# xyfJASON/diffusion-models-pytorch

Measured on AMD Instinct MI355X. Metric: images/sec at DDIM-50, CIFAR-10 UNet 32×32, bs=256; 1/2/4/8 GPU, higher is better.
Workload: dtype f32 via fp16x2 split MFMA

## Files before the change

diffusion-models-pytorch_amd/csrc/api.hip:

```cpp
#include <algorithm>
#include <cstdlib>
#include <cstring>
#include <string>
#include "dm_common.h"
#include "dm_kernels.h"

namespace dm {
namespace {
thread_local std::string g_last_error;
}
void set_error(const std::string& msg) { g_last_error = msg; }
const char* last_error() { return g_last_error.c_str(); }

namespace {
thread_local Toggles t_toggles;
thread_local const Toggles* t_scope = nullptr;
bool env_is(const char* name, char c) {
  const char* e = std::getenv(name);
  return e && e[0] == c;
}
bool g_launch_log_on = false;
bool g_launch_log_convs = false;
std::string g_launch_log;
}
// ... 16 lines not shown
  t.k32_small = !env_is("DM_CONV_K32S", '0');
  t.k32_s2 = !env_is("DM_CONV_K32S2", '0');
  t.k32_t2d = !env_is("DM_CONV_K32T2", '0');
  t.k32_8x = !env_is("DM_K32_8X", '0');
  t.gn_fusion = !env_is("DM_GN_FUSION", '0');
  if (const char* e = std::getenv("DM_ATTN")) {
    const std::string v(e);
    t.attn = v == "3" ? 3 : v == "0" || v == "presplit" ? 0 : v == "noproj" ? kAttnNoProj : v == "fused" ? kAttnFused
           : v == "unfused" ? kAttnUnfused : 4;
  }
  t.attn_gn_launch = env_is("DM_ATTN_GNFIN", '1');
  t.attn_small = !env_is("DM_ATTN_SMALL", '0');
  t.dit_presplit = !env_is("DM_DIT_PRESPLIT", '0');
  t.lin_sk = !env_is("DM_LIN_SK", '0');
  t.lin_rows = !env_is("DM_LIN_ROWS", '0');
  t_toggles = t;
}
void note_launch(const char* name) {
  if (!g_launch_log_on) return;
  g_launch_log += name;
  g_launch_log += '\n';
}
}

extern "C" int dm_debug_launch_log(int enable) {
  dm::g_launch_log_on = enable != 0;
  dm::g_launch_log_convs = enable == 2;
  if (enable) dm::g_launch_log.clear();
  return DM_OK;
}
// ... 309 lines not shown
```

diffusion-models-pytorch_amd/csrc/dm_kernels.h:

```cpp
#pragma once
#include <cstdlib>
#include <string>
#include "dm_common.h"

namespace dm {

constexpr int kGnPixPerChunk = 64;

constexpr int kAttnNoProj = 1, kAttnFused = 2, kAttnUnfused = 5;
struct Toggles {
  int conv_math = 2;
  bool range_check = true;
  bool graph = true;
  bool wino = true;
  bool k32s_w4 = false;
  bool k32_small = true;
  bool k32_s2 = true;
  bool k32_t2d = true;
  bool k32_8x = true;
  bool gn_fusion = true;
  int attn = 4;
  bool attn_gn_launch = false;
  bool attn_small = true;
  bool dit_presplit = true;
  bool lin_sk = true;
  bool lin_rows = true;
};
const Toggles& toggles();
void refresh_toggles();
const Toggles* toggle_scope_swap(const Toggles* t);
struct ToggleScope {
  const Toggles* prev;
  explicit ToggleScope(const Toggles& t) : prev(toggle_scope_swap(&t)) {}
  ~ToggleScope() { toggle_scope_swap(prev); }
  ToggleScope(const ToggleScope&) = delete;
  ToggleScope& operator=(const ToggleScope&) = delete;
};
void note_launch(const char* name);

constexpr int kPickBatch = 256;

// ... 340 lines not shown
```

diffusion-models-pytorch_amd/csrc/unet_exec.hip:

```cpp
#include <memory>
#include <vector>
#include <functional>
#include <cmath>
#include <map>
#include <set>

#include "dm_common.h"
#include "dm_kernels.h"
#include "plan.h"
#include "exec_pack.h"
#include "exec_core.h"

namespace dm {

namespace {

struct GnP { size_t g, b; int C; };
struct ConvP {
  size_t w, bias;
  int Cout, Cin, taps, K;
  size_t w_sub = 0;
};

struct ResBlockP {
// ... 50 lines not shown
  std::vector<AttnP> attn;
  std::vector<ConvP> convs;
  std::vector<Node> nodes;
  std::vector<int> skip_C, skip_level;
  int n_levels = 0;
  float norm_eps = 1e-5f;

  struct Plan : PlanBase {
    int B = 0, H = 0, W = 0;
    int math = 0;
    bool half = false;
    float* x = nullptr;
    int64_t* t = nullptr;
    int64_t* y = nullptr;
    float* out = nullptr;
  };
  PlanCache<Plan> plans;
  float* last_packed = nullptr;
  using FoldW = AttnFoldW;
  std::map<size_t, FoldW> folds;
  std::vector<void*> fold_mem;
  const FoldW* fold_for(const AttnP& p);

  UNetModel() { wino_small = true; }
  ~UNetModel() {
    for (void* q : fold_mem) (void)hipFree(q);
    if (last_packed) (void)hipFree(last_packed);
  }
  int build_plan(Plan& pl, int B, int H, int W);
  int get_plan(int B, int H, int W, int math, Plan** out) {
    conv_math = math;
    const bool half = half_active();
    return plans.get([&](const Plan& p) { return p.B == B && p.H == H && p.W == W && p.math == math && p.half == half; },
                     [&](Plan& p) { return build_plan(p, B, H, W); }, out);
  }
};

const UNetModel::FoldW* UNetModel::fold_for(const AttnP& p) {
  auto it = folds.find(p.wqkv);
  if (it != folds.end()) return it->second.at ? &it->second : nullptr;
  const int C = p.C;
  FoldW f;
  void* mem = nullptr;
  const size_t nb = attn_fold_bytes(C);
  if (hipMalloc(&mem, nb) != hipSuccess) {
    (void)hipGetLastError();
    folds[p.wqkv] = FoldW{};
    return nullptr;
  }
  fold_mem.push_back(mem);
  const double s = (double)p.sa * (p.sb != 0.f ? (double)p.sb : 1.0);
  if (attn_fold_all(P(p.wqkv), P(p.bqkv), P(p.wproj), P(p.bproj), C, s, mem, &f, nullptr) != DM_OK ||
      hipDeviceSynchronize() != hipSuccess) {
    folds[p.wqkv] = FoldW{};
    return nullptr;
  }
  split_bytes += nb - 64;
  return &(folds[p.wqkv] = f);
}

static int first_channels(const dm_unet_arch& a) { return a.variant == 2 ? a.dim * a.dim_mults[0] : a.dim; }

static int attn_heads(const dm_unet_arch& a, int C, int where) {
  if (a.variant == 3) return 1;
  if (a.variant == 2) {
    if (a.attn_head_dims > 0) return C / a.attn_head_dims;
    return where == 2 ? a.n_heads_up : a.n_heads;
  }
  if (where == 1) return 1;
  return a.variant == 1 ? C / a.attn_head_dims : a.n_heads;
}

static int count_params(const dm_unet_arch& a) {
// ... 385 lines not shown
  auto alloc = [&](size_t bytes) -> float* { return pl.alloc(bytes); };
  auto Hl = [&](int lvl) { return H >> lvl; };
  auto Wl = [&](int lvl) { return W >> lvl; };
  const int D = arch.dim, TD = 4 * arch.dim, G = 32, C0 = skip_C[0];
  const float gn_eps = norm_eps;

  pl.x = alloc((size_t)B * arch.in_channels * H * W * 4);
  pl.t = (int64_t*)alloc((size_t)B * 8);
  pl.y = (int64_t*)alloc((size_t)B * 8);
  pl.out = alloc((size_t)B * arch.out_channels * H * W * 4);
  float* e0 = alloc((size_t)B * D * 4);
  float* e1 = alloc((size_t)B * TD * 4);
  float* se = alloc((size_t)B * TD * 4);
  float* e2 = has_class ? alloc((size_t)B * TD * 4) : nullptr;
  float* projs = alloc((size_t)B * proj_total * 4);

  size_t max_a1 = 0, max_h = 0, max_attn = 0, max_qkv = 0, max_S = 0, max_xr = 0;
  int max_chunks = 1;
  for (auto& n : nodes) {
    const size_t hw = (size_t)Hl(n.level_in) * Wl(n.level_in);
    max_chunks = std::max(max_chunks, gn_num_chunks((int)hw));
    if (n.kind == N_RES) {
      const size_t hw_o = (size_t)Hl(n.level_out) * Wl(n.level_out);
      max_chunks = std::max(max_chunks, gn_num_chunks((int)hw_o));
      max_a1 = std::max(max_a1, (size_t)B * std::max(hw, hw_o) * n.cin);
      max_h = std::max(max_h, (size_t)B * hw_o * n.cout);
      if (res[n.idx].updown) max_xr = std::max(max_xr, (size_t)B * hw_o * n.cin);
    } else if (n.kind == N_ATTN) {
      max_attn = std::max(max_attn, (size_t)B * hw * n.cin);
      max_qkv = std::max(max_qkv, (size_t)B * hw * 3 * n.cin);
// ... 107 lines not shown
    conv_cost(c, fl, by);
    add(conv_label(c), fl, by, [=](hipStream_t st) { return conv2d_igemm(c, st); });
  };
  auto add_gemm = [&](const GemmArgs& g) {
    double fl, by;
    gemm_cost(g, fl, by);
    add(gemm_label(g), fl, by, [=](hipStream_t st) { return gemm_batched(g, st); });
  };
  auto gn_bytes = [](const View& v, bool apply) {
    const double n = (double)v.B * v.H * v.W * v.C;
    return apply ? 8.0 * n : 4.0 * n;
  };
  Plan* P_ = &pl;
  UNetModel* self = this;

  add("timestep_embed", 0, 4.0 * B * D, [=](hipStream_t st) {
    return timestep_embed(P_->t, B, D, self->arch.variant == 2 ? 1 : 0,
                          self->freqs_set ? self->P(self->freqs) : nullptr, e0, st);
  });
  auto add_rows = [&](const GemmArgs& g) {
    const long tiles64 = (long)ceil_div(kPickBatch, 64) * ceil_div(g.N, 64);
    if (!toggles().lin_rows || !linear_rows_ok(g) || tiles64 >= 256) return add_gemm(g);
    double fl, by;
    gemm_cost(g, fl, by);
    add("linear_rows_kernel", fl, by, [=](hipStream_t st) { return linear_rows(g, st); });
  };
  {
    GemmArgs g{};
    g.M = B; g.N = TD; g.K = D; g.Z1 = 1; g.Z2 = 1; g.pick_M = kPickBatch;
    g.A = e0; g.lda = D; g.Bm = P(te_w1); g.ldb = D; g.C = e1; g.ldc = TD; g.alpha = 1.f;
// ... 5 lines not shown
    if (has_class) {
      g2.act = 0;
      g2.C = e2;
      add_rows(g2);
      const float* table = P(class_embed);
      add("class_embed_silu", 0, 8.0 * B * TD, [=](hipStream_t st) {
        return embed_add_silu(e2, P_->y, table, B, TD, se, st);
      });
    } else {
      add_rows(g2);
    }
    GemmArgs g3 = g;
    g3.N = proj_total; g3.K = TD; g3.A = se; g3.lda = TD; g3.Bm = P(proj_w); g3.ldb = TD; g3.C = projs;
    g3.ldc = proj_total; g3.bias = P(proj_b); g3.act = 0;
    add_rows(g3);
  }

  auto out_view_for = [&](int i, int C, int lvl) -> View {
    if (i >= 0 && nodes[i].skip_producer) return skip_view[nodes[i].skip_id];
    const int nx = i + 1;
    if (nx < (int)nodes.size() && nodes[nx].kind == N_RES && nodes[nx].pops_skip >= 0) return concat_x[nx];
    float* buf = alloc((size_t)B * Hl(lvl) * Wl(lvl) * C * 4);
    return View{buf, B, Hl(lvl), Wl(lvl), C, C};
  };

  struct GnReady {
    double2* p;
    int C, G;
  };
  std::map<const float*, GnReady> gn_ready;
// ... 115 lines not shown
      View vh{hbuf, B, Ho, Wo, r.cout, r.cout};
      View va2{a2, B, Ho, Wo, r.cout, r.cout};
      View xres = xin;
      if (r.updown) {
        xres = View{xr, B, Ho, Wo, r.cin, r.cin};
        const bool down = r.updown == 2;
        add("resample2x", 0, 4.0 * B * ((double)Hi * Wi + (double)Ho * Wo) * r.cin,
            [=](hipStream_t st) { return resample2x(xin, xres, down, nullptr, nullptr, st); });
      }
      ConvArgs c1{};
      c1.x1_pitch = r.cin; c1.Cin1 = r.cin; c1.Hin = Ho; c1.Win = Wo;
      c1.taps = 9; c1.stride = 1; c1.upsample = 0;
      c1.w = P(r.conv1.w); c1.K = r.conv1.K;
      c1.y = hbuf; c1.y_pitch = r.cout; c1.Cout = r.cout; c1.B = B; c1.pick_B = kPickBatch; c1.Hout = Ho; c1.Wout = Wo;
      c1.bias = P(r.conv1.bias);
      if (!r.adagn) { c1.rowvec = projs + r.proj_col; c1.rowvec_pitch = proj_total; }
      if (r.updown == 1) { c1.upsample = 1; c1.Hin = Hi; c1.Win = Wi; }
      auto try_subpix = [&](ConvArgs& c, size_t w_sub) {
        if (!c.upsample || !w_sub) return;
        ConvArgs s = c;
        s.upsample = 2; s.w = P(w_sub); s.K = 4 * c.Cin1;
        split_for(s);
        if (conv_pick(s) >= 3) c = s;
      };
      ConvArgs c2{};
      c2.x1 = a2; c2.x1_pitch = r.cout; c2.Cin1 = r.cout; c2.Hin = Ho; c2.Win = Wo;
      c2.taps = 9; c2.stride = 1;
      c2.w = P(r.conv2.w); c2.K = r.conv2.K;
      c2.y = y.p; c2.y_pitch = y.pitch; c2.Cout = r.cout; c2.B = B; c2.pick_B = kPickBatch; c2.Hout = Ho; c2.Wout = Wo;
      c2.bias = P(r.conv2.bias);
      if (r.cin != r.cout) {
        c2.x2 = xres.p; c2.x2_pitch = xres.pitch; c2.Cin2 = r.cin;
      } else {
        c2.res = xres.p; c2.res_pitch = xres.pitch;
      }
      split_for(c1);
      split_for(c2);
      try_subpix(c1, r.conv1.w_sub);
      const bool fuse1 = r.updown != 2 && conv_pick(c1) >= 3, fuse2 = conv_pick(c2) >= 3;
      const float* ms = r.adagn ? projs + r.proj_col : nullptr;
      const float* mb = r.adagn ? projs + r.proj_col + r.cout : nullptr;
      const int mp = r.adagn ? proj_total : 0;
      const double2* st1 = n.pops_skip >= 0 ? gn_stats_concat(xin, skip_view[n.pops_skip]) : gn_stats(xin);
      if (r.updown && !fuse1) {
        add("gn_finalize", 0, 8.0 * B * r.cin, [=](hipStream_t st) {
          return gn_finalize(xin, G, st1, gn_eps, self->P(r.gn1.g), self->P(r.gn1.b), gsc, gsh, st);
        });
        const bool down = r.updown == 2;
        add("resample2x", 0, 4.0 * B * ((double)Hi * Wi + (double)Ho * Wo) * r.cin,
            [=](hipStream_t st) { return resample2x(xin, va1, down, gsc, gsh, st); });
        c1.x1 = a1; c1.upsample = 0; c1.Hin = Ho; c1.Win = Wo;
        c1.w = P(r.conv1.w); c1.K = r.conv1.K;
      } else if (fuse1) {
        c1.x1 = xin.p; c1.x1_pitch = xin.pitch;
        gn_prologue(c1, xin, st1, r.gn1.g, r.gn1.b, nullptr, nullptr, 0);
      } else {
        add("gn_apply", 0, gn_bytes(xin, true), [=](hipStream_t st) {
// ... 305 lines not shown
    for (int i = 0; i < n; ++i) order[i] = i;
  }
  return DM_OK;
}

extern "C" int dm_unet_create(const dm_unet_arch* arch, const float* const* params, const int64_t* numels,
                              int n_params, void* stream, dm_unet** out) {
  if (!out || !params || !numels) { dm::set_error("null argument"); return DM_ERR_ARG; }
  dm::UNetModel* m = nullptr;
  int rc = dm::unet_create(arch, params, numels, n_params, (hipStream_t)stream, &m);
  if (rc) return rc;
  *out = new dm_unet{m};
  return DM_OK;
}

extern "C" int dm_unet_forward(dm_unet* h, const float* x, const int64_t* t, const int64_t* y, int B, int H, int W,
                               float* out, void* stream) {
  dm::UNetModel* m = dm::model_of(h);
  DM_ABI_MODEL(m);
  if (!x || !t || !out) { dm::set_error("null tensor"); return DM_ERR_ARG; }
  if (B <= 0 || H <= 0 || W <= 0) { dm::set_error("empty batch or image"); return DM_ERR_ARG; }
  if (static_cast<const void*>(out) == static_cast<const void*>(x)) {
    dm::set_error("out must not alias x");
    return DM_ERR_ARG;
  }
  hipStream_t st = (hipStream_t)stream;
  const size_t nx = (size_t)B * m->arch.in_channels * H * W, no = (size_t)B * m->arch.out_channels * H * W;
  using Plan = dm::UNetModel::Plan;
  return dm::run_forward(
      *m, st, [&](int math, Plan** pl) { return m->get_plan(B, H, W, math, pl); },
      [&](Plan& pl) {
        DM_CHECK_HIP(hipMemcpyAsync(pl.x, x, nx * sizeof(float), hipMemcpyDeviceToDevice, st));
        DM_CHECK_HIP(hipMemcpyAsync(pl.t, t, (size_t)B * sizeof(int64_t), hipMemcpyDeviceToDevice, st));
        if (m->has_class) {
          if (y)
            DM_CHECK_HIP(hipMemcpyAsync(pl.y, y, (size_t)B * sizeof(int64_t), hipMemcpyDeviceToDevice, st));
          else
            DM_CHECK_HIP(hipMemsetAsync(pl.y, 0xff, (size_t)B * sizeof(int64_t), st));
        }
        return DM_OK;
      },
      [&](Plan& pl) {
        DM_CHECK_HIP(hipMemcpyAsync(out, pl.out, no * sizeof(float), hipMemcpyDeviceToDevice, st));
        return DM_OK;
      });
}

extern "C" int dm_unet_set_range_deferred(dm_unet* h, int deferred) {
  return dm::abi_set_range_deferred(dm::model_of(h), deferred);
}
extern "C" int dm_unet_range_poll(dm_unet* h, void* stream, int* flagged) {
  return dm::abi_range_poll(dm::model_of(h), (hipStream_t)stream, flagged);
}
extern "C" int dm_unet_range_fallback(dm_unet* h, int on) { return dm::abi_range_fallback(dm::model_of(h), on); }
extern "C" int dm_unet_range_stats(const dm_unet* h, int64_t* fallbacks, int* active) {
  return dm::abi_range_stats(dm::model_of(h), fallbacks, active);
}
extern "C" int dm_unet_memory(const dm_unet* h, int64_t* weight_bytes, int64_t* workspace_bytes) {
  return dm::abi_memory(dm::model_of(h), weight_bytes, workspace_bytes);
}

extern "C" int dm_unet_share_workspace(dm_unet* a, dm_unet* b) {
  if (!a || !a->m || !b || !b->m) { dm::set_error("null model"); return DM_ERR_STATE; }
  if (a->m->plans.pool != b->m->plans.pool) b->m->plans.share(a->m->plans.pool);
  return DM_OK;
}

extern "C" int dm_unet_plan_stats(const dm_unet* h, int64_t* builds, int* cached) {
  return dm::abi_plan_stats(dm::model_of(h), builds, cached);
}
extern "C" int dm_unet_set_conv_math(dm_unet* h, int kind) { return dm::abi_set_math(dm::model_of(h), kind, true); }
extern "C" int dm_unet_get_conv_math(const dm_unet* h, int* kind) { return dm::abi_get_math(dm::model_of(h), kind); }

extern "C" int dm_unet_set_conv_half(dm_unet* h, int on) {
  auto* m = dm::model_of(h);
  DM_ABI_MODEL(m);
  if (on != 0 && on != 1) { dm::set_error("conv_half must be 0 or 1"); return DM_ERR_ARG; }
  if ((on != 0) != m->conv_half) {
    m->conv_half = on != 0;
    m->plans.clear();
  }
  return DM_OK;
}
extern "C" int dm_unet_get_conv_half(const dm_unet* h, int* on) {
  auto* m = dm::model_of(h);
  DM_ABI_MODEL(m && on);
  *on = m->conv_half ? 1 : 0;
  return DM_OK;
}
extern "C" int dm_unet_set_time_freqs(dm_unet* h, const float* freqs, int n, void* stream) {
  return dm::abi_set_time_freqs(dm::model_of(h), freqs, n, (hipStream_t)stream);
}
extern "C" int dm_unet_profile(dm_unet* h, int enable) { return dm::abi_profile(dm::model_of(h), enable); }
extern "C" int dm_unet_profile_count(dm_unet* h, int* n_ops) { return dm::abi_profile_count(dm::model_of(h), n_ops); }
extern "C" int dm_unet_profile_get(dm_unet* h, int i, char* label, int label_len, double* flops, double* bytes,
                                   double* ms_total, int64_t* launches) {
  return dm::abi_profile_get(dm::model_of(h), i, label, label_len, flops, bytes, ms_total, launches);
}
extern "C" void dm_unet_destroy(dm_unet* h) { dm::abi_destroy(h); }
```

diffusion-models-pytorch_amd/diffusions/ddim.py:

```python
from typing import Any, Dict

import torch
import tqdm
from torch import Tensor

from diffusions.ddpm import DDPM, _CFGMixin


class DDIM(DDPM):
    kind = 0

    def __init__(
            self,
            total_steps: int = 1000,
            beta_schedule: str = 'linear',
            beta_start: float = 0.0001,
            beta_end: float = 0.02,
            betas: Tensor = None,
            objective: str = 'pred_eps',

            clip_denoised: bool = True,
            respace_type: str = None,
            respace_steps: int = 100,
            respaced_seq: Tensor = None,
# ... 34 lines not shown
        if self.eta != 0.:
            raise ValueError(f'DDIM inversion is only valid when eta=0, get {self.eta}')
        out = self._step(model_output, xt, t, 0, model_output_uncond=model_output_uncond,
                         guidance_scale=guidance_scale, want_noise=False, coefs=self._inversion_coefs(t, t_next))
        return {'sample': out['sample'], 'pred_x0': out['pred_x0'], 'pred_eps': out['pred_eps']}

    def sample_inversion_loop(
            self, model, img: Tensor,
            tqdm_kwargs: Dict = None, model_kwargs: Dict = None,
    ):
        tqdm_kwargs = dict() if tqdm_kwargs is None else tqdm_kwargs
        model_kwargs = dict() if model_kwargs is None else model_kwargs
        seq = self.respaced_seq.tolist()
        pbar = tqdm.tqdm(total=len(seq) - 1, **tqdm_kwargs)
        for t, t_next in zip(seq[:-1], seq[1:]):
            t_batch = torch.full((img.shape[0], ), t, device=img.device, dtype=torch.long)
            model_output = model(img, t_batch, **model_kwargs)
            out = self.denoise_inversion(model_output, img, t, t_next)
            img = out['sample']
            pbar.update(1)
            yield out
        pbar.close()

    def sample_inversion(
            self, model, img: Tensor,
            tqdm_kwargs: Dict = None, model_kwargs: Dict = None,
    ):
        sample = None
        for out in self.sample_inversion_loop(model, img, tqdm_kwargs, model_kwargs):
            sample = out['sample']
        return sample

# ... 40 lines not shown
```

diffusion-models-pytorch_amd/diffusions/ddpm.py:

```python
import math
from contextlib import contextmanager
from typing import Any, Callable, Dict, Optional

import torch
import tqdm
from torch import Tensor

import dmhip
from diffusions.schedule import get_beta_schedule, get_respaced_seq

_OBJECTIVES = {'pred_eps': 0, 'pred_x0': 1, 'pred_v': 2}
_VAR_TYPES = ('fixed_small', 'fixed_large', 'learned_range')


class DDPM:
    kind = 1

    def __init__(
            self,
            total_steps: int = 1000,
            beta_schedule: str = 'linear',
            beta_start: float = 0.0001,
            beta_end: float = 0.02,
            betas: Tensor = None,
            objective: str = 'pred_eps',

            var_type: str = 'fixed_large',
# ... 214 lines not shown

    def denoise(self, model_output: Tensor, xt: Tensor, t: int, t_prev: int):
        return self._step(model_output, xt, t, t_prev)

    def sample_loop(
            self, model, init_noise: Tensor,
            tqdm_kwargs: Dict = None, model_kwargs: Dict = None,
    ):
        tqdm_kwargs = dict() if tqdm_kwargs is None else tqdm_kwargs
        model_kwargs = dict() if model_kwargs is None else model_kwargs
        img = init_noise
        seq = self.respaced_seq.tolist()
        seq_prev = [-1] + seq[:-1]
        pbar = tqdm.tqdm(total=len(seq), **tqdm_kwargs)
        for t, t_prev in zip(reversed(seq), reversed(seq_prev)):
            t_batch = torch.full((img.shape[0], ), t, device=img.device, dtype=torch.long)
            model_output = model(img, t_batch, **model_kwargs)
            out = self.denoise(model_output, img, t, t_prev)
            img = out['sample']
            pbar.update(1)
            yield out
        pbar.close()

    def sample(
            self, model, init_noise: Tensor,
            tqdm_kwargs: Dict = None, model_kwargs: Dict = None,
    ):
        def run():
            sample = None
            for out in self.sample_loop(model, init_noise, tqdm_kwargs, model_kwargs):
                sample = out['sample']
            return sample
# ... 87 lines not shown
```

diffusion-models-pytorch_amd/diffusions/heun.py:

```python
from typing import Dict

import torch
import tqdm
from torch import Tensor

from diffusions.euler import EulerSampler


class HeunSampler(EulerSampler):
    def __init__(self, *args, **kwargs):
        super().__init__(*args, **kwargs)
        self._1st_order_derivative = None
        self._1st_order_xt = None

    def denoise_1st_order(self, model_output: Tensor, xt: Tensor, t: int, t_prev: int):
        derivative = torch.empty_like(xt)
        out = self._first_order(model_output, xt, t, t_prev, derivative=derivative)
        self._1st_order_derivative = derivative
        self._1st_order_xt = xt
        return {'sample': out['sample'], 'pred_x0': out['pred_x0']}

    def denoise_2nd_order(self, model_output: Tensor, xt_prev: Tensor, t: int, t_prev: int):
        if self._1st_order_derivative is None:
            raise RuntimeError('denoise_2nd_order needs a preceding denoise_1st_order')
# ... 5 lines not shown
        self._1st_order_derivative = None
        self._1st_order_xt = None
        return {'sample': out['sample'], 'pred_x0': out['pred_x0']}

    def sample_loop(
            self, model, init_noise: Tensor,
            tqdm_kwargs: Dict = None, model_kwargs: Dict = None,
    ):
        tqdm_kwargs = dict() if tqdm_kwargs is None else tqdm_kwargs
        model_kwargs = dict() if model_kwargs is None else model_kwargs
        img = init_noise
        seq = self.respaced_seq.tolist()
        seq_prev = [-1] + seq[:-1]
        pbar = tqdm.tqdm(total=len(seq), **tqdm_kwargs)
        for t, t_prev in zip(reversed(seq), reversed(seq_prev)):
            t_batch = torch.full((img.shape[0], ), t, device=img.device, dtype=torch.long)
            model_output = model(img, t_batch, **model_kwargs)
            out = self.denoise_1st_order(model_output, img, t, t_prev)
            img = out['sample']
            if t_prev >= 0:
                t_prev_batch = torch.full((img.shape[0], ), t_prev, device=img.device, dtype=torch.long)
                model_output = model(img, t_prev_batch, **model_kwargs)
                out = self.denoise_2nd_order(model_output, img, t, t_prev)
                img = out['sample']
            pbar.update(1)
            yield out
        pbar.close()
```

diffusion-models-pytorch_amd/dmhip/__init__.py:

```python
from dmhip._lib import (
    DMError,
    lib,
    lib_path,
    load,
    exported_symbols,
    require_device_tensor,
    stream_handle,
    StepDesc,
    ConvDesc,
    GemmDesc,
    UNetArch,
    DiTArch,
    VaeArch,
    VaeEncArch,
    sampler_step,
    groupnorm_nhwc,
    groupnorm_affine,
    conv2d_nhwc,
    conv2d_nhwc_s2pad0,
    conv2d_gn_stats,
    pack_conv_weight,
    pack_conv_weight_subpixel,
    pack_conv_weight_split,
    pack_conv_weight_wino,
# ... 8 lines not shown
    SPLIT_BF16X3,
    MATH_FP16,
    MATH_NAMES,
    TOKEN_MATH,
    gemm,
    softmax_rows,
    timestep_embedding,
    unet_profile_enable,
    unet_profile_read,
    null_label_scope,
    null_labels_allowed,
    deferred_range_check,
    plan_stats,
    range_stats,
    share_workspace,
    lincomb,
    GuideDesc,
    guided_step,
    LowpassPlan,
)
```

diffusion-models-pytorch_amd/dmhip/_lib.py:

```python
import ctypes
import os
import re
from typing import Optional

import torch

_HERE = os.path.dirname(os.path.abspath(__file__))
lib_path = os.environ.get('DM_HIP_LIB') or os.path.join(_HERE, 'libdm_hip.so')
_HEADER = os.path.join(os.path.dirname(os.path.dirname(_HERE)), 'include', 'dm_hip.h')

ABI_VERSION = 2
DM_OK = 0
DM_ERR_ARG = -1
DM_ERR_HIP = -2
DM_ERR_STATE = -3
DM_ERR_UNSUPPORTED = -4
DM_MAX_STAGES = 8


class DMError(RuntimeError):
    """A failure reported by the native library (HIP error, bad state)."""


c_float_p = ctypes.POINTER(ctypes.c_float)
# ... 191 lines not shown

    def end_fallback(self):
        for handle, abi in self.flagged_handles:
            check(getattr(load(), abi + '_range_fallback')(handle, 0), abi + '_range_fallback')
        self.flagged_handles = []


def _declare(L: ctypes.CDLL):
    L.dm_abi_version.restype = ctypes.c_int
    L.dm_last_error.restype = ctypes.c_char_p
    L.dm_build_info.restype = ctypes.c_char_p
    L.dm_unet_param_count.argtypes = [ctypes.POINTER(UNetArch), ctypes.POINTER(ctypes.c_int)]
    L.dm_unet_create.argtypes = [ctypes.POINTER(UNetArch), ctypes.POINTER(vp), ctypes.POINTER(ctypes.c_int64),
                                 ctypes.c_int, vp, ctypes.POINTER(vp)]
    L.dm_unet_forward.argtypes = [vp, vp, vp, vp, ctypes.c_int, ctypes.c_int, ctypes.c_int, vp, vp]
    L.dm_unet_profile.argtypes = [vp, ctypes.c_int]
    L.dm_unet_profile_count.argtypes = [vp, ctypes.POINTER(ctypes.c_int)]
    L.dm_unet_profile_get.argtypes = [vp, ctypes.c_int, ctypes.c_char_p, ctypes.c_int,
                                      ctypes.POINTER(ctypes.c_double), ctypes.POINTER(ctypes.c_double),
                                      ctypes.POINTER(ctypes.c_double), ctypes.POINTER(ctypes.c_int64)]
    L.dm_unet_memory.argtypes = [vp, ctypes.POINTER(ctypes.c_int64), ctypes.POINTER(ctypes.c_int64)]
    L.dm_unet_destroy.argtypes = [vp]
    L.dm_unet_destroy.restype = None
    L.dm_sampler_step.argtypes = [ctypes.POINTER(StepDesc), vp]
    L.dm_groupnorm_scratch_bytes.argtypes = [ctypes.c_int, ctypes.c_int, ctypes.c_int]
    L.dm_groupnorm_scratch_bytes.restype = ctypes.c_int64
    L.dm_groupnorm_nhwc.argtypes = [vp, ctypes.c_int, vp, ctypes.c_int, ctypes.c_int, ctypes.c_int, ctypes.c_int,
                                    ctypes.c_int, ctypes.c_float, vp, vp, vp, vp, ctypes.c_int, ctypes.c_int, vp, vp]
    L.dm_groupnorm_affine.argtypes = [vp, ctypes.c_int, ctypes.c_int, ctypes.c_int, ctypes.c_int, ctypes.c_int,
                                      ctypes.c_float, vp, vp, vp, vp, vp, vp]
# ... 391 lines not shown


def range_stats(handle, abi: str = 'dm_unet'):
    n, active = ctypes.c_int64(), ctypes.c_int()
    check(getattr(load(), abi + '_range_stats')(handle, ctypes.byref(n), ctypes.byref(active)), abi + '_range_stats')
    return n.value, {v: k for k, v in MATH_NAMES.items()}[active.value]


def plan_stats(handle, abi: str = 'dm_unet'):
    builds, cached = ctypes.c_int64(), ctypes.c_int()
    check(getattr(load(), abi + '_plan_stats')(handle, ctypes.byref(builds), ctypes.byref(cached)),
          abi + '_plan_stats')
    return builds.value, cached.value


def share_workspace(a, b):
    check(load().dm_unet_share_workspace(a, b), 'dm_unet_share_workspace')


def lincomb(mode: int, a: torch.Tensor, b: torch.Tensor, c1, c2, out: torch.Tensor = None) -> torch.Tensor:
    for name, t in (('a', a), ('b', b)):
        require_device_tensor(t, name)
    if a.shape != b.shape:
        raise ValueError(f'lincomb: shapes {tuple(a.shape)} and {tuple(b.shape)} differ')
    if out is None:
        out = torch.empty_like(a)
    else:
        require_device_tensor(out, 'out')
        if out.shape != a.shape:
            raise ValueError(f'lincomb: out has shape {tuple(out.shape)}, the operands {tuple(a.shape)}')
# ... 34 lines not shown
```

diffusion-models-pytorch_amd/models/pesser/model.py:

```python
from typing import Sequence

import torch.nn as nn
from torch import Tensor

from ..unet import ConvHalf, NativeDenoiser


def _gn(C: int) -> nn.GroupNorm:
    return nn.GroupNorm(32, C, eps=1e-6)


def _conv(cin: int, cout: int, k: int, stride: int = 1, padding: int = None) -> nn.Conv2d:
    return nn.Conv2d(cin, cout, k, stride=stride, padding=k // 2 if padding is None else padding)


def _holder(**children) -> nn.Module:
    m = nn.Module()
    for name, child in children.items():
        m.add_module(name, child)
    return m


class ResnetBlock(nn.Module):

# ... 13 lines not shown
    def __init__(self, C: int):
        super().__init__()
        self.norm = _gn(C)
        for name in ('q', 'k', 'v', 'proj_out'):
            self.add_module(name, _conv(C, C, 1))


class Resample(nn.Module):

    def __init__(self, C: int, down: bool):
        super().__init__()
        self.conv = _conv(C, C, 3, stride=2, padding=0) if down else _conv(C, C, 3)


class Model(ConvHalf, NativeDenoiser):
    def __init__(self, *, ch: int, out_ch: int, ch_mult: Sequence[int] = (1, 2, 4, 8), num_res_blocks: int,
                 attn_resolutions: Sequence[int], dropout: float = 0.0, resamp_with_conv: bool = True,
                 in_channels: int, resolution: int):
        super().__init__()
        if not resamp_with_conv:
            raise NotImplementedError('resamp_with_conv=False (average-pool / nearest resampling without convs) is '
                                      'used by no shipped config and is not built')
        self.ch = ch
        self.resolution = resolution
        self.in_channels = in_channels
        listed = {int(r) for r in attn_resolutions}
        widths = [ch * int(m) for m in ch_mult]
        n_levels = len(widths)
        use_attn = [(resolution >> lvl) in listed for lvl in range(n_levels)]
        self.arch = dict(in_channels=in_channels, out_channels=out_ch, dim=ch, dim_mults=[int(m) for m in ch_mult],
# ... 23 lines not shown
                           block_2=ResnetBlock(cur, cur, embed))

        ups = {}
        for lvl in reversed(range(n_levels)):
            cins = []
            for _ in range(num_res_blocks + 1):
                cins.append(cur + skips.pop())
                cur = widths[lvl]
            ups[lvl] = stage(lvl, cins, dict(upsample=Resample(cur, down=False)) if lvl else {})
        assert not skips
        self.up = nn.ModuleList(ups[lvl] for lvl in range(n_levels))

        self.norm_out = _gn(cur)
        self.conv_out = _conv(cur, out_ch, 3)

    def forward(self, x: Tensor, t: Tensor):
        if tuple(x.shape[2:]) != (self.resolution, self.resolution):
            raise AssertionError(f'expected {self.resolution} x {self.resolution} images, got {tuple(x.shape[2:])}')
        return self._run(x, t)
```

diffusion-models-pytorch_amd/models/unet.py:

```python
import ctypes
import math
from typing import List, Sequence

import torch
import torch.nn as nn
from torch import Tensor

import dmhip
from dmhip._lib import UNetArch, check, load, stream_handle


def _gn(C: int) -> nn.GroupNorm:
    return nn.GroupNorm(32, C)


def _conv(cin: int, cout: int, k: int, stride: int = 1) -> nn.Conv2d:
    return nn.Conv2d(cin, cout, k, stride=stride, padding=k // 2)


class ResBlock(nn.Module):

    def __init__(self, in_channels: int, out_channels: int, embed_dim: int, dropout: float = 0.1):
        super().__init__()
        self.blk1 = nn.Sequential(_gn(in_channels), nn.SiLU(), _conv(in_channels, out_channels, 3))
# ... 17 lines not shown
        self.scale = (dim // n_heads) ** -0.5


class _TimeEmbedding(nn.Sequential):

    def __init__(self, dim: int):
        super().__init__(nn.Identity(), nn.Linear(dim, 4 * dim), nn.SiLU(), nn.Linear(4 * dim, 4 * dim))


class NativeDenoiser(nn.Module):

    _native = None
    _native_key = None
    _param_list = None
    _abi = 'dm_unet'

    def _arch_struct(self) -> UNetArch:
        a = UNetArch()
        a.in_channels = self.arch['in_channels']
        a.out_channels = self.arch['out_channels']
        a.dim = self.arch['dim']
        a.n_stages = len(self.arch['dim_mults'])
        for i, (m, at) in enumerate(zip(self.arch['dim_mults'], self.arch['use_attn'])):
            a.dim_mults[i] = m
            a.use_attn[i] = int(at)
        a.num_res_blocks = self.arch['num_res_blocks']
        a.n_heads = self.arch.get('n_heads', 1)
        a.variant = self.arch.get('variant', 0)
        a.num_classes = self.arch.get('num_classes', 0) or 0
        a.attn_head_dims = self.arch.get('attn_head_dims', 0)
# ... 55 lines not shown
        if peer is not None and self._abi == 'dm_unet' and getattr(peer, '_abi', None) == 'dm_unet' \
                and getattr(peer, '_native', None) is not None:
            dmhip.share_workspace(peer._native, handle)

    def _time_freqs(self) -> Tensor:
        half = self.arch['dim'] // 2
        if self.arch.get('variant', 0) == 2:
            return torch.exp(-math.log(10000) * torch.arange(start=0, end=half, dtype=torch.float32) / half)
        return torch.exp(torch.arange(half) * -(math.log(10000) / (half - 1)))

    def _launch(self, handle, X: Tensor, T: Tensor, y_ptr, out: Tensor):
        B, _, H, W = X.shape
        check(load().dm_unet_forward(handle, X.data_ptr(), T.data_ptr(), y_ptr, B, H, W, out.data_ptr(),
                                     stream_handle(X.device)), 'dm_unet_forward')

    def _apply(self, fn, *args, **kwargs):
        self._release_native()
        return super()._apply(fn, *args, **kwargs)

    def __del__(self):
        try:
            self._release_native()
        except Exception:
            pass

    def _run(self, X: Tensor, T: Tensor, y: Tensor = None) -> Tensor:
        dmhip.require_device_tensor(X, 'X')
        dmhip.require_device_tensor(T, 'T', dtype=torch.long)
        if X.ndim != 4 or X.shape[1] != self.arch['in_channels']:
            raise ValueError(f'expected input [B, {self.arch["in_channels"]}, H, W], got {tuple(X.shape)}')
        B, _, H, W = X.shape
        if T.shape != (B, ):
            raise ValueError(f'expected T of shape ({B},), got {tuple(T.shape)}')
        y_ptr = None
        if y is not None:
            dmhip.require_device_tensor(y, 'y', dtype=torch.long)
            if y.shape != (B, ):
                raise ValueError(f'expected y of shape ({B},), got {tuple(y.shape)}')
            self._check_labels(y)
            y_ptr = y.data_ptr()
        handle = self.native_handle(X.device)
        scope = dmhip.deferred_range_check.active
        if scope is not None:
            scope.register(handle, self._abi, X.device)
        out = torch.empty((B, self.arch['out_channels'], H, W), device=X.device, dtype=torch.float32)
        self._launch(handle, X, T, y_ptr, out)
        return out

    def _check_labels(self, y: Tensor):
        null_ok = dmhip.null_labels_allowed()
        key = (y.data_ptr(), y._version, y.numel(), null_ok)
        if getattr(self, '_labels_ok', None) == key:
            return
        n = self.arch.get('label_rows', self.arch.get('num_classes', 0) or 0)
        if y.numel():
            hi, lo = int(y.max()), int(y.min())
            if hi >= n:
                raise IndexError(f'class label {hi} out of range for num_classes={n}')
            if lo < (-1 if null_ok else 0):
                raise IndexError(f'class label {lo} out of range for num_classes={n}')
        self._labels_ok = key
# ... 6 lines not shown
    def set_conv_half(self, on: bool = True) -> bool:
        self._conv_half = bool(on)
        if self._native is not None:
            dmhip.unet_conv_half(self._native, self._conv_half)
        return self._conv_half

    def native_handle(self, device: torch.device):
        had = self._native
        handle = super().native_handle(device)
        if handle is not had and self._conv_half is not None:
            dmhip.unet_conv_half(handle, self._conv_half)
        return handle


class UNet(ConvHalf, NativeDenoiser):
    def __init__(
            self,
            in_channels: int = 3,
            out_channels: int = 3,
            dim: int = 128,
            dim_mults: List[int] = (1, 2, 2, 2),
            use_attn: List[int] = (False, True, False, False),
            num_res_blocks: int = 2,
            n_heads: int = 1,
            dropout: float = 0.1,
    ):
        super().__init__()
        if len(dim_mults) != len(use_attn):
            raise ValueError('dim_mults and use_attn must have the same length')
        self.arch = dict(in_channels=in_channels, out_channels=out_channels, dim=dim,
# ... 27 lines not shown
        self.up_blocks = nn.ModuleList()
        for i in reversed(range(len(dim_mults))):
            out = dim * dim_mults[i]
            stage = nn.ModuleList()
            for _ in range(num_res_blocks + 1):
                stage.append(ResBlock(chans.pop() + cur, out, temb, dropout))
                if use_attn[i]:
                    stage.append(SelfAttentionBlock(out, n_heads=n_heads))
                cur = out
            if i > 0:
                stage.append(nn.Sequential(nn.Upsample(scale_factor=2, mode='nearest'), _conv(out, out, 3)))
            self.up_blocks.append(stage)

        self.last_conv = nn.Sequential(_gn(cur), nn.SiLU(), _conv(cur, out_channels, 3))

    def forward(self, X: Tensor, T: Tensor):
        return self._run(X, T)
```

include/dm_hip.h:

```cpp
#ifndef DM_HIP_H_
#define DM_HIP_H_

#include <stdint.h>

#ifdef __cplusplus
extern "C" {
#endif

#define DM_ABI_VERSION 2

#define DM_OK 0
#define DM_ERR_ARG (-1)
#define DM_ERR_HIP (-2)
#define DM_ERR_STATE (-3)
#define DM_ERR_UNSUPPORTED (-4)

int dm_abi_version(void);
const char* dm_build_info(void);
const char* dm_last_error(void);

#define DM_MAX_STAGES 8
typedef struct dm_unet_arch {
  int in_channels;
  int out_channels;
// ... 8 lines not shown
  int attn_head_dims;
  int resblock_updown;
  int n_heads_up;
  int scale_shift_norm;
  int pool_resample;
  int attn_legacy;
} dm_unet_arch;

typedef struct dm_unet dm_unet;

int dm_unet_param_count(const dm_unet_arch* arch, int* n_params);
int dm_unet_create(const dm_unet_arch* arch, const float* const* params, const int64_t* numels,
                   int n_params, void* stream, dm_unet** out);
int dm_unet_forward(dm_unet* m, const float* x, const int64_t* t, const int64_t* y, int B, int H, int W,
                    float* out, void* stream);
int dm_unet_set_time_freqs(dm_unet* m, const float* freqs, int n, void* stream);
int dm_unet_profile(dm_unet* m, int enable);
int dm_unet_profile_count(dm_unet* m, int* n_ops);
int dm_unet_profile_get(dm_unet* m, int i, char* label, int label_len, double* flops, double* bytes,
                        double* ms_total, int64_t* launches);
int dm_unet_memory(const dm_unet* m, int64_t* weight_bytes, int64_t* workspace_bytes);
int dm_unet_share_workspace(dm_unet* a, dm_unet* b);
int dm_unet_plan_stats(const dm_unet* m, int64_t* builds, int* cached);
int dm_unet_set_conv_math(dm_unet* m, int kind);
int dm_unet_get_conv_math(const dm_unet* m, int* kind);
int dm_unet_set_conv_half(dm_unet* m, int on);
int dm_unet_get_conv_half(const dm_unet* m, int* on);
int dm_unet_set_range_deferred(dm_unet* m, int deferred);
int dm_unet_range_poll(dm_unet* m, void* stream, int* flagged);
int dm_unet_range_fallback(dm_unet* m, int on);
// ... 267 lines not shown
```

Measured before the change: 712.9.

## Add uniform-timestep forward path with cached per-timestep embedding projection rows

Adds a forward entry point that takes a single scalar timestep for the whole batch, used by the DDIM/DDPM/Heun samplers when the model supports it. In this mode the timestep-embedding MLP and the per-block projection chain are taken out of the main plan. They are run only when a timestep is first seen, and the resulting single projection row is kept in a device-side LRU cache keyed by timestep. Convolutions and adaptive group-norm then read that row with a zero batch pitch. This removes the per-step embedding work, the per-step host tensor creation, and the per-batch projection reads, at the cost of extra cache state. That state must be invalidated whenever weights, frequencies or math mode change.

```diff
diff --git a/diffusion-models-pytorch_amd/csrc/api.hip b/diffusion-models-pytorch_amd/csrc/api.hip
--- a/diffusion-models-pytorch_amd/csrc/api.hip
+++ b/diffusion-models-pytorch_amd/csrc/api.hip
@@ -54,6 +54,7 @@
   t.dit_presplit = !env_is("DM_DIT_PRESPLIT", '0');
   t.lin_sk = !env_is("DM_LIN_SK", '0');
   t.lin_rows = !env_is("DM_LIN_ROWS", '0');
+  t.uniform_t = !env_is("DM_UNIFORM_T", '0');
   t_toggles = t;
 }
 void note_launch(const char* name) {
diff --git a/diffusion-models-pytorch_amd/csrc/dm_kernels.h b/diffusion-models-pytorch_amd/csrc/dm_kernels.h
--- a/diffusion-models-pytorch_amd/csrc/dm_kernels.h
+++ b/diffusion-models-pytorch_amd/csrc/dm_kernels.h
@@ -25,6 +25,7 @@
   bool dit_presplit = true;
   bool lin_sk = true;
   bool lin_rows = true;
+  bool uniform_t = true;
 };
 const Toggles& toggles();
 void refresh_toggles();
diff --git a/diffusion-models-pytorch_amd/csrc/unet_exec.hip b/diffusion-models-pytorch_amd/csrc/unet_exec.hip
--- a/diffusion-models-pytorch_amd/csrc/unet_exec.hip
+++ b/diffusion-models-pytorch_amd/csrc/unet_exec.hip
@@ -88,8 +88,60 @@
     int64_t* t = nullptr;
     int64_t* y = nullptr;
     float* out = nullptr;
+    bool uniform = false;
+    std::vector<Op> chain;
+    float* projs = nullptr;
+    float* trow = nullptr;
   };
   PlanCache<Plan> plans;
+  struct UtCache {
+    static constexpr int kMaxRows = 1024;
+    float* rows = nullptr;
+    int limit = kMaxRows;
+    std::map<int64_t, int> slot_of;
+    std::vector<int64_t> t_of;
+    std::vector<uint64_t> used;
+    uint64_t tick = 0;
+    int64_t hits = 0, misses = 0, evictions = 0;
+    void clear() {
+      slot_of.clear();
+      t_of.clear();
+      used.clear();
+    }
+    void release() {
+      clear();
+      if (rows) {
+        (void)hipDeviceSynchronize();
+        (void)hipFree(rows);
+      }
+      rows = nullptr;
+    }
+    int find(int64_t t) {
+      auto it = slot_of.find(t);
+      if (it == slot_of.end()) return -1;
+      used[it->second] = ++tick;
+      return it->second;
+    }
+    int take(int64_t t) {
+      int s = (int)t_of.size();
+      if (s < limit) {
+        t_of.push_back(t);
+        used.push_back(0);
+      } else {
+        s = (int)(std::min_element(used.begin(), used.end()) - used.begin());
+        slot_of.erase(t_of[s]);
+        t_of[s] = t;
+        ++evictions;
+      }
+      slot_of[t] = s;
+      used[s] = ++tick;
+      return s;
+    }
+  } ut;
+  void drop_plans() {
+    plans.clear();
+    ut.clear();
+  }
   float* last_packed = nullptr;
   using FoldW = AttnFoldW;
   std::map<size_t, FoldW> folds;
@@ -100,14 +152,23 @@
   ~UNetModel() {
     for (void* q : fold_mem) (void)hipFree(q);
     if (last_packed) (void)hipFree(last_packed);
+    ut.release();
   }
   int build_plan(Plan& pl, int B, int H, int W);
-  int get_plan(int B, int H, int W, int math, Plan** out) {
+  int get_plan(int B, int H, int W, int math, Plan** out, bool uniform = false) {
     conv_math = math;
     const bool half = half_active();
-    return plans.get([&](const Plan& p) { return p.B == B && p.H == H && p.W == W && p.math == math && p.half == half; },
-                     [&](Plan& p) { return build_plan(p, B, H, W); }, out);
-  }
+    return plans.get(
+        [&](const Plan& p) {
+          return p.B == B && p.H == H && p.W == W && p.math == math && p.half == half && p.uniform == uniform;
+        },
+        [&](Plan& p) {
+          p.uniform = uniform;
+          return build_plan(p, B, H, W);
+        },
+        out);
+  }
+  int stage_trow(Plan& pl, int64_t t, hipStream_t st);
 };
 
 const UNetModel::FoldW* UNetModel::fold_for(const AttnP& p) {
@@ -131,6 +192,52 @@
   }
   split_bytes += nb - 64;
   return &(folds[p.wqkv] = f);
+}
+
+namespace {
+__global__ void fill_timestep_kernel(int64_t* __restrict__ t, int B, int64_t v) {
+  const int b = blockIdx.x * blockDim.x + threadIdx.x;
+  if (b < B) t[b] = v;
+}
+int fill_timestep(int64_t* t, int B, int64_t v, hipStream_t st) {
+  hipLaunchKernelGGL(fill_timestep_kernel, dim3(ceil_div(B, 256)), dim3(256), 0, st, t, B, v);
+  DM_LAUNCH_CHECK();
+  return DM_OK;
+}
+}
+
+int UNetModel::stage_trow(Plan& pl, int64_t t, hipStream_t st) {
+  const size_t row_bytes = (size_t)proj_total * sizeof(float);
+  int slot = ut.find(t);
+  if (slot >= 0) {
+    ++ut.hits;
+  } else {
+    if (!ut.rows) {
+      void* p = nullptr;
+      if (hipMalloc(&p, (size_t)UtCache::kMaxRows * row_bytes) != hipSuccess) {
+        (void)hipGetLastError();
+        set_error("timestep row cache allocation failed");
+        return DM_ERR_HIP;
+      }
+      ut.rows = static_cast<float*>(p);
+    }
+    if (const int rc = fill_timestep(pl.t, pl.B, t, st)) return rc;
+    {
+      ToggleScope scope(pl.toggles);
+      for (auto& op : pl.chain)
+        if (const int rc = op.fn(st)) return rc;
+    }
+    slot = ut.take(t);
+    ++ut.misses;
+    const hipError_t e = hipMemcpyAsync(ut.rows + (size_t)slot * proj_total, pl.projs, row_bytes,
+                                        hipMemcpyDeviceToDevice, st);
+    if (e != hipSuccess) {
+      ut.clear();
+      DM_CHECK_HIP(e);
+    }
+  }
+  DM_CHECK_HIP(hipMemcpyAsync(pl.trow, ut.rows + (size_t)slot * proj_total, row_bytes, hipMemcpyDeviceToDevice, st));
+  return DM_OK;
 }
 
 static int first_channels(const dm_unet_arch& a) { return a.variant == 2 ? a.dim * a.dim_mults[0] : a.dim; }
@@ -546,6 +653,10 @@
   float* se = alloc((size_t)B * TD * 4);
   float* e2 = has_class ? alloc((size_t)B * TD * 4) : nullptr;
   float* projs = alloc((size_t)B * proj_total * 4);
+  pl.projs = projs;
+  if (pl.uniform) pl.trow = alloc((size_t)proj_total * 4);
+  const float* tproj = pl.uniform ? pl.trow : projs;
+  const int tpitch = pl.uniform ? 0 : proj_total;
 
   size_t max_a1 = 0, max_h = 0, max_attn = 0, max_qkv = 0, max_S = 0, max_xr = 0;
   int max_chunks = 1;
@@ -683,6 +794,7 @@
   Plan* P_ = &pl;
   UNetModel* self = this;
 
+  const size_t ops_before_chain = pl.ops.size();
   add("timestep_embed", 0, 4.0 * B * D, [=](hipStream_t st) {
     return timestep_embed(P_->t, B, D, self->arch.variant == 2 ? 1 : 0,
                           self->freqs_set ? self->P(self->freqs) : nullptr, e0, st);
@@ -718,6 +830,10 @@
     g3.N = proj_total; g3.K = TD; g3.A = se; g3.lda = TD; g3.Bm = P(proj_w); g3.ldb = TD; g3.C = projs;
     g3.ldc = proj_total; g3.bias = P(proj_b); g3.act = 0;
     add_rows(g3);
+  }
+  if (pl.uniform) {
+    pl.chain.assign(pl.ops.begin() + ops_before_chain, pl.ops.end());
+    pl.ops.erase(pl.ops.begin() + ops_before_chain, pl.ops.end());
   }
 
   auto out_view_for = [&](int i, int C, int lvl) -> View {
@@ -863,7 +979,7 @@
       c1.w = P(r.conv1.w); c1.K = r.conv1.K;
       c1.y = hbuf; c1.y_pitch = r.cout; c1.Cout = r.cout; c1.B = B; c1.pick_B = kPickBatch; c1.Hout = Ho; c1.Wout = Wo;
       c1.bias = P(r.conv1.bias);
-      if (!r.adagn) { c1.rowvec = projs + r.proj_col; c1.rowvec_pitch = proj_total; }
+      if (!r.adagn) { c1.rowvec = tproj + r.proj_col; c1.rowvec_pitch = tpitch; }
       if (r.updown == 1) { c1.upsample = 1; c1.Hin = Hi; c1.Win = Wi; }
       auto try_subpix = [&](ConvArgs& c, size_t w_sub) {
         if (!c.upsample || !w_sub) return;
@@ -887,9 +1003,9 @@
       split_for(c2);
       try_subpix(c1, r.conv1.w_sub);
       const bool fuse1 = r.updown != 2 && conv_pick(c1) >= 3, fuse2 = conv_pick(c2) >= 3;
-      const float* ms = r.adagn ? projs + r.proj_col : nullptr;
-      const float* mb = r.adagn ? projs + r.proj_col + r.cout : nullptr;
-      const int mp = r.adagn ? proj_total : 0;
+      const float* ms = r.adagn ? tproj + r.proj_col : nullptr;
+      const float* mb = r.adagn ? tproj + r.proj_col + r.cout : nullptr;
+      const int mp = r.adagn ? tpitch : 0;
       const double2* st1 = n.pops_skip >= 0 ? gn_stats_concat(xin, skip_view[n.pops_skip]) : gn_stats(xin);
       if (r.updown && !fuse1) {
         add("gn_finalize", 0, 8.0 * B * r.cin, [=](hipStream_t st) {
@@ -1225,24 +1341,32 @@
   return DM_OK;
 }
 
-extern "C" int dm_unet_forward(dm_unet* h, const float* x, const int64_t* t, const int64_t* y, int B, int H, int W,
-                               float* out, void* stream) {
-  dm::UNetModel* m = dm::model_of(h);
-  DM_ABI_MODEL(m);
-  if (!x || !t || !out) { dm::set_error("null tensor"); return DM_ERR_ARG; }
+static int unet_forward(dm::UNetModel* m, const float* x, const int64_t* t, int64_t t_all, const int64_t* y, int B,
+                        int H, int W, float* out, hipStream_t st) {
+  if (!x || !out) { dm::set_error("null tensor"); return DM_ERR_ARG; }
   if (B <= 0 || H <= 0 || W <= 0) { dm::set_error("empty batch or image"); return DM_ERR_ARG; }
   if (static_cast<const void*>(out) == static_cast<const void*>(x)) {
     dm::set_error("out must not alias x");
     return DM_ERR_ARG;
   }
-  hipStream_t st = (hipStream_t)stream;
+  bool uniform = false;
+  if (!t) {
+    dm::refresh_toggles();
+    uniform = !m->has_class && dm::toggles().uniform_t;
+  }
   const size_t nx = (size_t)B * m->arch.in_channels * H * W, no = (size_t)B * m->arch.out_channels * H * W;
   using Plan = dm::UNetModel::Plan;
   return dm::run_forward(
-      *m, st, [&](int math, Plan** pl) { return m->get_plan(B, H, W, math, pl); },
+      *m, st, [&](int math, Plan** pl) { return m->get_plan(B, H, W, math, pl, uniform); },
       [&](Plan& pl) {
         DM_CHECK_HIP(hipMemcpyAsync(pl.x, x, nx * sizeof(float), hipMemcpyDeviceToDevice, st));
-        DM_CHECK_HIP(hipMemcpyAsync(pl.t, t, (size_t)B * sizeof(int64_t), hipMemcpyDeviceToDevice, st));
+        if (uniform) {
+          if (const int rc = m->stage_trow(pl, t_all, st)) return rc;
+        } else if (t) {
+          DM_CHECK_HIP(hipMemcpyAsync(pl.t, t, (size_t)B * sizeof(int64_t), hipMemcpyDeviceToDevice, st));
+        } else if (const int rc = dm::fill_timestep(pl.t, B, t_all, st)) {
+          return rc;
+        }
         if (m->has_class) {
           if (y)
             DM_CHECK_HIP(hipMemcpyAsync(pl.y, y, (size_t)B * sizeof(int64_t), hipMemcpyDeviceToDevice, st));
@@ -1257,6 +1381,40 @@
       });
 }
 
+extern "C" int dm_unet_forward(dm_unet* h, const float* x, const int64_t* t, const int64_t* y, int B, int H, int W,
+                               float* out, void* stream) {
+  dm::UNetModel* m = dm::model_of(h);
+  DM_ABI_MODEL(m);
+  if (!t) { dm::set_error("null tensor"); return DM_ERR_ARG; }
+  return unet_forward(m, x, t, 0, y, B, H, W, out, (hipStream_t)stream);
+}
+
+extern "C" int dm_unet_forward_ut(dm_unet* h, const float* x, int64_t t, const int64_t* y, int B, int H, int W,
+                                  float* out, void* stream) {
+  dm::UNetModel* m = dm::model_of(h);
+  DM_ABI_MODEL(m);
+  return unet_forward(m, x, nullptr, t, y, B, H, W, out, (hipStream_t)stream);
+}
+
+extern "C" int dm_unet_ut_stats(const dm_unet* h, int64_t* hits, int64_t* misses, int64_t* evictions, int* rows) {
+  const dm::UNetModel* m = dm::model_of(h);
+  DM_ABI_MODEL(m);
+  if (hits) *hits = m->ut.hits;
+  if (misses) *misses = m->ut.misses;
+  if (evictions) *evictions = m->ut.evictions;
+  if (rows) *rows = (int)m->ut.t_of.size();
+  return DM_OK;
+}
+
+extern "C" int dm_debug_unet_ut_limit(dm_unet* h, int rows) {
+  dm::UNetModel* m = dm::model_of(h);
+  DM_ABI_MODEL(m);
+  if (rows < 0 || rows > dm::UNetModel::UtCache::kMaxRows) { dm::set_error("row bound out of range"); return DM_ERR_ARG; }
+  m->ut.limit = rows ? rows : dm::UNetModel::UtCache::kMaxRows;
+  m->ut.clear();
+  return DM_OK;
+}
+
 extern "C" int dm_unet_set_range_deferred(dm_unet* h, int deferred) {
   return dm::abi_set_range_deferred(dm::model_of(h), deferred);
 }
@@ -1273,14 +1431,23 @@
 
 extern "C" int dm_unet_share_workspace(dm_unet* a, dm_unet* b) {
   if (!a || !a->m || !b || !b->m) { dm::set_error("null model"); return DM_ERR_STATE; }
-  if (a->m->plans.pool != b->m->plans.pool) b->m->plans.share(a->m->plans.pool);
+  if (a->m->plans.pool != b->m->plans.pool) {
+    b->m->plans.share(a->m->plans.pool);
+    b->m->ut.clear();
+  }
   return DM_OK;
 }
 
 extern "C" int dm_unet_plan_stats(const dm_unet* h, int64_t* builds, int* cached) {
   return dm::abi_plan_stats(dm::model_of(h), builds, cached);
 }
-extern "C" int dm_unet_set_conv_math(dm_unet* h, int kind) { return dm::abi_set_math(dm::model_of(h), kind, true); }
+extern "C" int dm_unet_set_conv_math(dm_unet* h, int kind) {
+  auto* m = dm::model_of(h);
+  const int before = m ? m->base_math : 0;
+  const int rc = dm::abi_set_math(m, kind, true);
+  if (m && m->base_math != before) m->ut.clear();
+  return rc;
+}
 extern "C" int dm_unet_get_conv_math(const dm_unet* h, int* kind) { return dm::abi_get_math(dm::model_of(h), kind); }
 
 extern "C" int dm_unet_set_conv_half(dm_unet* h, int on) {
@@ -1289,7 +1456,7 @@
   if (on != 0 && on != 1) { dm::set_error("conv_half must be 0 or 1"); return DM_ERR_ARG; }
   if ((on != 0) != m->conv_half) {
     m->conv_half = on != 0;
-    m->plans.clear();
+    m->drop_plans();
   }
   return DM_OK;
 }
@@ -1300,7 +1467,9 @@
   return DM_OK;
 }
 extern "C" int dm_unet_set_time_freqs(dm_unet* h, const float* freqs, int n, void* stream) {
-  return dm::abi_set_time_freqs(dm::model_of(h), freqs, n, (hipStream_t)stream);
+  auto* m = dm::model_of(h);
+  if (m) m->ut.clear();
+  return dm::abi_set_time_freqs(m, freqs, n, (hipStream_t)stream);
 }
 extern "C" int dm_unet_profile(dm_unet* h, int enable) { return dm::abi_profile(dm::model_of(h), enable); }
 extern "C" int dm_unet_profile_count(dm_unet* h, int* n_ops) { return dm::abi_profile_count(dm::model_of(h), n_ops); }
diff --git a/diffusion-models-pytorch_amd/diffusions/ddim.py b/diffusion-models-pytorch_amd/diffusions/ddim.py
--- a/diffusion-models-pytorch_amd/diffusions/ddim.py
+++ b/diffusion-models-pytorch_amd/diffusions/ddim.py
@@ -4,7 +4,7 @@
 import tqdm
 from torch import Tensor
 
-from diffusions.ddpm import DDPM, _CFGMixin
+from diffusions.ddpm import DDPM, _CFGMixin, timestep_arg
 
 
 class DDIM(DDPM):
@@ -72,8 +72,7 @@
         seq = self.respaced_seq.tolist()
         pbar = tqdm.tqdm(total=len(seq) - 1, **tqdm_kwargs)
         for t, t_next in zip(seq[:-1], seq[1:]):
-            t_batch = torch.full((img.shape[0], ), t, device=img.device, dtype=torch.long)
-            model_output = model(img, t_batch, **model_kwargs)
+            model_output = model(img, timestep_arg(model, t, img), **model_kwargs)
             out = self.denoise_inversion(model_output, img, t, t_next)
             img = out['sample']
             pbar.update(1)
diff --git a/diffusion-models-pytorch_amd/diffusions/ddpm.py b/diffusion-models-pytorch_amd/diffusions/ddpm.py
--- a/diffusion-models-pytorch_amd/diffusions/ddpm.py
+++ b/diffusion-models-pytorch_amd/diffusions/ddpm.py
@@ -11,6 +11,12 @@
 
 _OBJECTIVES = {'pred_eps': 0, 'pred_x0': 1, 'pred_v': 2}
 _VAR_TYPES = ('fixed_small', 'fixed_large', 'learned_range')
+
+
+def timestep_arg(model, t: int, img: Tensor):
+    if getattr(model, 'uniform_timestep', False):
+        return int(t)
+    return torch.full((img.shape[0], ), t, device=img.device, dtype=torch.long)
 
 
 class DDPM:
@@ -255,8 +261,7 @@
         seq_prev = [-1] + seq[:-1]
         pbar = tqdm.tqdm(total=len(seq), **tqdm_kwargs)
         for t, t_prev in zip(reversed(seq), reversed(seq_prev)):
-            t_batch = torch.full((img.shape[0], ), t, device=img.device, dtype=torch.long)
-            model_output = model(img, t_batch, **model_kwargs)
+            model_output = model(img, timestep_arg(model, t, img), **model_kwargs)
             out = self.denoise(model_output, img, t, t_prev)
             img = out['sample']
             pbar.update(1)
diff --git a/diffusion-models-pytorch_amd/diffusions/heun.py b/diffusion-models-pytorch_amd/diffusions/heun.py
--- a/diffusion-models-pytorch_amd/diffusions/heun.py
+++ b/diffusion-models-pytorch_amd/diffusions/heun.py
@@ -4,6 +4,7 @@
 import tqdm
 from torch import Tensor
 
+from diffusions.ddpm import timestep_arg
 from diffusions.euler import EulerSampler
 
 
@@ -43,13 +44,11 @@
         seq_prev = [-1] + seq[:-1]
         pbar = tqdm.tqdm(total=len(seq), **tqdm_kwargs)
         for t, t_prev in zip(reversed(seq), reversed(seq_prev)):
-            t_batch = torch.full((img.shape[0], ), t, device=img.device, dtype=torch.long)
-            model_output = model(img, t_batch, **model_kwargs)
+            model_output = model(img, timestep_arg(model, t, img), **model_kwargs)
             out = self.denoise_1st_order(model_output, img, t, t_prev)
             img = out['sample']
             if t_prev >= 0:
-                t_prev_batch = torch.full((img.shape[0], ), t_prev, device=img.device, dtype=torch.long)
-                model_output = model(img, t_prev_batch, **model_kwargs)
+                model_output = model(img, timestep_arg(model, t_prev, img), **model_kwargs)
                 out = self.denoise_2nd_order(model_output, img, t, t_prev)
                 img = out['sample']
             pbar.update(1)
diff --git a/diffusion-models-pytorch_amd/dmhip/__init__.py b/diffusion-models-pytorch_amd/dmhip/__init__.py
--- a/diffusion-models-pytorch_amd/dmhip/__init__.py
+++ b/diffusion-models-pytorch_amd/dmhip/__init__.py
@@ -46,6 +46,8 @@
     plan_stats,
     range_stats,
     share_workspace,
+    uniform_t_stats,
+    uniform_t_limit,
     lincomb,
     GuideDesc,
     guided_step,
diff --git a/diffusion-models-pytorch_amd/dmhip/_lib.py b/diffusion-models-pytorch_amd/dmhip/_lib.py
--- a/diffusion-models-pytorch_amd/dmhip/_lib.py
+++ b/diffusion-models-pytorch_amd/dmhip/_lib.py
@@ -229,6 +229,10 @@
     L.dm_unet_create.argtypes = [ctypes.POINTER(UNetArch), ctypes.POINTER(vp), ctypes.POINTER(ctypes.c_int64),
                                  ctypes.c_int, vp, ctypes.POINTER(vp)]
     L.dm_unet_forward.argtypes = [vp, vp, vp, vp, ctypes.c_int, ctypes.c_int, ctypes.c_int, vp, vp]
+    if hasattr(L, 'dm_unet_forward_ut'):
+        L.dm_unet_forward_ut.argtypes = [vp, vp, ctypes.c_int64, vp, ctypes.c_int, ctypes.c_int, ctypes.c_int, vp, vp]
+        L.dm_unet_ut_stats.argtypes = [vp] + [ctypes.POINTER(ctypes.c_int64)] * 3 + [ctypes.POINTER(ctypes.c_int)]
+        L.dm_debug_unet_ut_limit.argtypes = [vp, ctypes.c_int]
     L.dm_unet_profile.argtypes = [vp, ctypes.c_int]
     L.dm_unet_profile_count.argtypes = [vp, ctypes.POINTER(ctypes.c_int)]
     L.dm_unet_profile_get.argtypes = [vp, ctypes.c_int, ctypes.c_char_p, ctypes.c_int,
@@ -650,6 +654,17 @@
     return builds.value, cached.value
 
 
+def uniform_t_stats(handle):
+    h, m, e, n = ctypes.c_int64(), ctypes.c_int64(), ctypes.c_int64(), ctypes.c_int()
+    check(load().dm_unet_ut_stats(handle, ctypes.byref(h), ctypes.byref(m), ctypes.byref(e), ctypes.byref(n)),
+          'dm_unet_ut_stats')
+    return h.value, m.value, e.value, n.value
+
+
+def uniform_t_limit(handle, rows: int):
+    check(load().dm_debug_unet_ut_limit(handle, rows), 'dm_debug_unet_ut_limit')
+
+
 def share_workspace(a, b):
     check(load().dm_unet_share_workspace(a, b), 'dm_unet_share_workspace')
 
diff --git a/diffusion-models-pytorch_amd/models/pesser/model.py b/diffusion-models-pytorch_amd/models/pesser/model.py
--- a/diffusion-models-pytorch_amd/models/pesser/model.py
+++ b/diffusion-models-pytorch_amd/models/pesser/model.py
@@ -51,6 +51,8 @@
 
 
 class Model(ConvHalf, NativeDenoiser):
+    uniform_timestep = True
+
     def __init__(self, *, ch: int, out_ch: int, ch_mult: Sequence[int] = (1, 2, 4, 8), num_res_blocks: int,
                  attn_resolutions: Sequence[int], dropout: float = 0.0, resamp_with_conv: bool = True,
                  in_channels: int, resolution: int):
@@ -104,7 +106,7 @@
         self.norm_out = _gn(cur)
         self.conv_out = _conv(cur, out_ch, 3)
 
-    def forward(self, x: Tensor, t: Tensor):
+    def forward(self, x: Tensor, t):
         if tuple(x.shape[2:]) != (self.resolution, self.resolution):
             raise AssertionError(f'expected {self.resolution} x {self.resolution} images, got {tuple(x.shape[2:])}')
         return self._run(x, t)
diff --git a/diffusion-models-pytorch_amd/models/unet.py b/diffusion-models-pytorch_amd/models/unet.py
--- a/diffusion-models-pytorch_amd/models/unet.py
+++ b/diffusion-models-pytorch_amd/models/unet.py
@@ -55,6 +55,7 @@
     _native_key = None
     _param_list = None
     _abi = 'dm_unet'
+    uniform_timestep = False
 
     def _arch_struct(self) -> UNetArch:
         a = UNetArch()
@@ -140,6 +141,11 @@
         check(load().dm_unet_forward(handle, X.data_ptr(), T.data_ptr(), y_ptr, B, H, W, out.data_ptr(),
                                      stream_handle(X.device)), 'dm_unet_forward')
 
+    def _launch_uniform(self, handle, X: Tensor, t: int, y_ptr, out: Tensor):
+        B, _, H, W = X.shape
+        check(load().dm_unet_forward_ut(handle, X.data_ptr(), t, y_ptr, B, H, W, out.data_ptr(),
+                                        stream_handle(X.device)), 'dm_unet_forward_ut')
+
     def _apply(self, fn, *args, **kwargs):
         self._release_native()
         return super()._apply(fn, *args, **kwargs)
@@ -150,14 +156,20 @@
         except Exception:
             pass
 
-    def _run(self, X: Tensor, T: Tensor, y: Tensor = None) -> Tensor:
+    def _run(self, X: Tensor, T, y: Tensor = None) -> Tensor:
         dmhip.require_device_tensor(X, 'X')
-        dmhip.require_device_tensor(T, 'T', dtype=torch.long)
         if X.ndim != 4 or X.shape[1] != self.arch['in_channels']:
             raise ValueError(f'expected input [B, {self.arch["in_channels"]}, H, W], got {tuple(X.shape)}')
         B, _, H, W = X.shape
-        if T.shape != (B, ):
-            raise ValueError(f'expected T of shape ({B},), got {tuple(T.shape)}')
+        uniform = isinstance(T, int) and not isinstance(T, bool)
+        if uniform and not self.uniform_timestep:
+            raise TypeError(f'{type(self).__name__} takes T as a [B] int64 tensor')
+        if uniform and not hasattr(load(), 'dm_unet_forward_ut'):
+            uniform, T = False, torch.full((B, ), T, device=X.device, dtype=torch.long)
+        if not uniform:
+            dmhip.require_device_tensor(T, 'T', dtype=torch.long)
+            if T.shape != (B, ):
+                raise ValueError(f'expected T of shape ({B},), got {tuple(T.shape)}')
         y_ptr = None
         if y is not None:
             dmhip.require_device_tensor(y, 'y', dtype=torch.long)
@@ -170,7 +182,10 @@
         if scope is not None:
             scope.register(handle, self._abi, X.device)
         out = torch.empty((B, self.arch['out_channels'], H, W), device=X.device, dtype=torch.float32)
-        self._launch(handle, X, T, y_ptr, out)
+        if uniform:
+            self._launch_uniform(handle, X, T, y_ptr, out)
+        else:
+            self._launch(handle, X, T, y_ptr, out)
         return out
 
     def _check_labels(self, y: Tensor):
@@ -207,6 +222,8 @@
 
 
 class UNet(ConvHalf, NativeDenoiser):
+    uniform_timestep = True
+
     def __init__(
             self,
             in_channels: int = 3,
@@ -264,5 +281,5 @@
 
         self.last_conv = nn.Sequential(_gn(cur), nn.SiLU(), _conv(cur, out_channels, 3))
 
-    def forward(self, X: Tensor, T: Tensor):
+    def forward(self, X: Tensor, T):
         return self._run(X, T)
diff --git a/include/dm_hip.h b/include/dm_hip.h
--- a/include/dm_hip.h
+++ b/include/dm_hip.h
@@ -46,6 +46,9 @@
                    int n_params, void* stream, dm_unet** out);
 int dm_unet_forward(dm_unet* m, const float* x, const int64_t* t, const int64_t* y, int B, int H, int W,
                     float* out, void* stream);
+int dm_unet_forward_ut(dm_unet* m, const float* x, int64_t t, const int64_t* y, int B, int H, int W, float* out,
+                       void* stream);
+int dm_unet_ut_stats(const dm_unet* m, int64_t* hits, int64_t* misses, int64_t* evictions, int* rows);
 int dm_unet_set_time_freqs(dm_unet* m, const float* freqs, int n, void* stream);
 int dm_unet_profile(dm_unet* m, int enable);
 int dm_unet_profile_count(dm_unet* m, int* n_ops);
```

Result: no change. 719.5, median of 6 (+0.9%).
